# jan-frost/uzliti_slam

Hardware: AMD Instinct MI355X
Metric: SE(3) edges optimized/sec (node-pairs matched/sec in `secondary`) (higher is better)
Workload: dtype f64; 1 GPU; BASELINE config 2: 1000-node / 5000-edge SE(3) pose graph, 20 LM iterations, Huber(1) on loop closures; one independent graph per GPU; system_edges=4999

## Files before the change

### uzliti_slam_amd/csrc/pgo_handle.hpp

```cpp
#pragma once
#include "uzl_common.hpp"
#include "pgo_types.hpp"
#include "pgo_schur.hpp"
#include "pgo_ml_plan.hpp"
#include "pgo_structure.hpp"
#include "pgo_lm.hpp"

#include <algorithm>
#include <chrono>
#include <cstdlib>
#include <cmath>
#include <functional>
#include <limits>
#include <new>
#include <numeric>

namespace uzl {
void k_prepare_nodes(const uzl_node* nodes, int n, int xy, double* pose, hipStream_t s);
void k_prepare_flat_nodes(const double* poses12, int n, double* pose, hipStream_t s);
void k_prepare_edges(const uzl_edge* edges, const int32_t* src, int e, const double* sensors, int ns, int xy, int odom_params,
                     double* zinv, double* info, hipStream_t s);
void k_prepare_flat_edges(const double* meas12, const double* info36, int e, double* zinv, double* info, hipStream_t s);
int k_chi2(const PgoDev& D, const double* pose, double delta, hipStream_t s);
int k_chi2_trial(const PgoDev& D, const double* pose, double delta, hipStream_t s);
// ... 20 lines not shown
void k_edge_error(const PgoDev& D, const double* pose, double* err, hipStream_t s);
void k_poses_out(const double* pose, int n, double* out12, hipStream_t s);
void k_schur_gather(const PgoDev& D, const SchurDev& S, hipStream_t s);
void k_lm_head(const LmSlot* slots, int nslots, int pass_flags, hipStream_t s);
void k_lm_tail(const LmSlot* slots, int nslots, hipStream_t s);
hipError_t kl_linearize(const LmSlot* sl, int nslots, int g_edges, int g_asm, hipStream_t s);
void kl_eval(const LmSlot* sl, int nslots, int g_edges, int g_oplus, hipStream_t s);
void kl_schur_reduce(const LmSlot* sl, const LmShape& sh, hipStream_t s);
void kl_schur_backsub(const LmSlot* sl, const LmShape& sh, hipStream_t s);
void kl_schur_reduce(const HostSlot& hs, const LmShape& sh, hipStream_t s, KernelTimer* timer);
void kl_schur_backsub(const HostSlot& hs, const LmShape& sh, hipStream_t s, KernelTimer* timer);
void kl_ml_numeric(const LmSlot* sl, const LmShape& sh, int which, hipStream_t s);
void kl_ml_trial(const LmSlot* sl, const LmShape& sh, int which, int ns_steps, hipStream_t s);
void kl_ml_numeric(const HostSlot& hs, const LmShape& sh, hipStream_t s, KernelTimer* timer, const std::function<void()>& level1_done);
void kl_ml_trial(const HostSlot& hs, const LmShape& sh, int ns_steps, hipStream_t s, KernelTimer* timer);
void ml_cg_variant(const MlHot& ml, int agg, size_t lds_full, int32_t* variant, int32_t* comp_u, uint64_t* lds);
hipError_t kl_ml_init(const LmSlot* sl, const LmSlot* by_value, const LmShape& sh, int ix, hipStream_t s);
hipError_t kl_ml_pcg_its(const LmSlot* sl, const LmSlot* by_value, const LmShape& sh, int ix, double tol2, int first, int n, hipStream_t s, hipEvent_t* ev = nullptr);
void kl_ml_pcg_init(const HostSlot& hs, const LmShape& sh, hipStream_t s);
void kl_ml_spmv(const HostSlot& hs, const LmShape& sh, int parity, hipStream_t s, hipEvent_t ev_a = nullptr, hipEvent_t ev_b = nullptr);
hipError_t kl_ml_cg(const HostSlot& hs, const LmShape& sh, int parity, int init, hipStream_t s, hipEvent_t ev_a = nullptr, hipEvent_t ev_b = nullptr);
}



namespace uzl { struct LmRun; }
using namespace uzl;

struct SysBufs {
    DevBuf<int32_t> row_ptr, col, rowhdr, b2v;
// ... 75 lines not shown
    struct MlBuf {
        MlDev* dml = nullptr;
        MlHot hot;
        double* rg[2] = {nullptr, nullptr};
        double* y1 = nullptr; double* nsT = nullptr; double* nsX = nullptr;
        double* l1_span_ptr = nullptr;
        hipGraph_t graph = nullptr; hipGraphExec_t graph_exec = nullptr;
        hipGraph_t graph_s = nullptr; hipGraphExec_t graph_exec_s = nullptr;
        double lambda_setup = 0.;
    } mlb[2];
    double* ml_dense_ptr[2][kMlMaxLevels + 1] = {};
    int ml_ix = 0;
    bool ml_pending = false;
    hipStream_t stream2 = nullptr;
    bool streams_borrowed = false;
    hipEvent_t ev_lin = nullptr, ev_setup = nullptr;
    DevBuf<double> d_scal2;
    double lambda_now = 0.;
    DevBuf<uint8_t> ml_arena;
    size_t ml_copy_stride = 0;
    DevBuf<MlDev> d_ml;
    bool no_graph = false;
    int32_t rank = 0, world = 1;
    uzl_allreduce_fn allreduce = nullptr;
    void* allreduce_user = nullptr;
    void* rccl_comm = nullptr;
    bool sharded = false;
    DevBuf<double> d_red;
    int64_t iter_span = 0;
    int64_t l1_span = 0;
    double structure_ms = 0., exchange_ms = 0.;
// ... 17 lines not shown
inline double pgo_eps_t(const uzl_pgo_cfg& c) { return c.pcg_stop == 1 ? 0. : kStepT * c.pcg_tol; }
inline double pgo_eps_r(const uzl_pgo_cfg& c) { return c.pcg_stop == 1 ? 0. : kStepR * c.pcg_tol; }
void build_structure(uzl_pgo* h);
void ensure_structure(uzl_pgo* h);
void destroy_pcg_graph(uzl_pgo* h);
bool ml_async_level(const uzl_pgo* h);
double ml_rate_drop(const uzl_pgo* h);
int ml_ns_steps_at(int structure_steps, int lm_iteration);
void prepare_optimize(uzl_pgo* h);
void own_streams(uzl_pgo* h, bool drain_borrowed);
int do_optimize_host(uzl_pgo* h, int32_t iterations, uzl_pgo_stats* st);
int do_optimize(uzl_pgo* h, int32_t iterations, uzl_pgo_stats* st);
HostSlot host_slot(uzl_pgo* h);
void set_lambda(uzl_pgo* h, double lambda, double tol_f2);
void ml_setup_numeric(uzl_pgo* h, const HostSlot& hs, hipStream_t s, KernelTimer* timer);
int pcg_solve(uzl_pgo* h, int it, bool* converged);
inline double tol_factor2(const uzl_pgo_cfg& c) { return pgo_tol_f2(c); }
struct LmRun;
void lm_run_destroy(LmRun* r);
bool lm_eligible(const uzl_pgo* h);
int do_optimize_lm(uzl_pgo* h, int32_t iterations, uzl_pgo_stats* st);
bool lm_batch_eligible(const std::vector<uzl_pgo*>& hs);
LmSlot make_slot(const uzl_pgo* h, LmDev* d_lm, LmHost* d_pub);
LmShape make_shape(const std::vector<uzl_pgo*>& hs, int nslots, bool batch_geometry);
int batch_optimize_lm(LmRun*& R, const std::vector<uzl_pgo*>& hs, int resident, hipStream_t s, hipStream_t s2, int32_t iterations, bool eager, bool verbose, KernelTimer* timer,
                      uzl_pgo_stats* stats, int* rc_all);
constexpr int kSchurStrongOneMax = 256;
extern const int kUpperNs;
constexpr double kRefreshRel = 1e-3;
constexpr double kRefreshRelSync = 3e-2;
constexpr double kLambdaRetake = 32.;
// ... 4 lines not shown
```

### uzliti_slam_amd/csrc/pgo_ml_kernels.hip

```cpp
#include <hip/hip_ext.h>
#include <functional>
#include <mutex>
#include <type_traits>

#include "pgo_device.hpp"
#include "uzl_common.hpp"

namespace uzl {

#ifdef UZL_STAMPS
__device__ unsigned long long g_stamps[64];
#define STAMP_DECL unsigned long long st_prev_ = __builtin_amdgcn_s_memrealtime(); int st_i_ = 0;
#define STAMP(base) do { if (blockIdx.x == 0 && threadIdx.x == 0) { unsigned long long n_ = __builtin_amdgcn_s_memrealtime(); \
        atomicAdd(&g_stamps[(base) + st_i_], n_ - st_prev_); st_prev_ = n_; } st_i_++; } while (0)
#else
#define STAMP_DECL
#define STAMP(base) do { } while (0)
#endif

struct P3 { double X[9], Y[9], Z[9]; };

__device__ __forceinline__ void mat3(const double* A, const double* B, double* C)
{
#pragma unroll
// ... 2126 lines not shown
    const int B = sh.nslots;
    if (timer) timer->begin("ml_geometry", s);
    if (sh.n_lv[1] <= kGeoAllMax) hipLaunchKernelGGL(ml_geometry_lm_kernel<SLOT>, dim3(1, 1, B), dim3(kBlk), 0, s, sl, which, 0);
    else
        for (int l = 1; l <= sh.levels; l++)
            hipLaunchKernelGGL(ml_geometry_lm_kernel<SLOT>, dim3((sh.n_lv[l] + kBlk - 1) / kBlk, 1, B), dim3(kBlk), 0, s, sl, which, l);
    if (timer) timer->end(s);
    for (int f = 0; f < sh.levels; f++) {
        if (timer) timer->begin("ml_galerkin", s);
        if (sh.chunks[f + 1] > 0) hipLaunchKernelGGL(ml_galerkin_lm_kernel<SLOT>, dim3(sh.chunks[f + 1], 1, B), dim3(kBlk), 0, s, sl, which, f);
        if (timer) timer->end(s);
        if (f == 0 && level1_done) level1_done();
    }
}
template <class SLOT>
static void kl_ml_trial_t(SLOT sl, const LmShape& sh, int which, int ns_steps, hipStream_t s, KernelTimer* timer)
{
    const int B = sh.nslots, L = sh.levels, cl = sh.cl;
    if (timer) timer->begin("ml_sibling", s);
    hipLaunchKernelGGL(ml_inverses_lm_kernel<SLOT>, dim3((sh.inner_aggs + kSibPerBlk - 1) / kSibPerBlk + 1, 1, B), dim3(kBlk), 0, s, sl, which);
    if (timer) timer->end(s);
    if (cl == 0) return;
    const int n6c = 6 * sh.n_lv[cl];
    const long work32 = (long)n6c * (((n6c + 3) & ~3) >> 2);
    if (timer) timer->begin("ml_dense", s);
    if (!sh.mult) {
        for (int l = L - 1; l >= cl; l--)
            hipLaunchKernelGGL(ml_dense_level_lm_kernel<SLOT>, dim3((sh.n_lv[l] * sh.n_lv[l] + kBlk - 1) / kBlk, 1, B), dim3(kBlk), 0, s, sl, which, l);
        hipLaunchKernelGGL(ml_cmat32_lm_kernel<SLOT>, dim3((unsigned)((work32 + kBlk - 1) / kBlk), 1, B), dim3(kBlk), 0, s, sl, which, cl);
        if (timer) timer->end(s);
        return;
    }
    for (int l = L - 1; l >= cl; l--) {
        const int n1 = sh.n_lv[l], n2 = sh.n_lv[l + 1];
        hipLaunchKernelGGL(ml_mult_pair_lm_kernel<SLOT>, dim3(n2 * n2, 1, B), dim3(kBlk), 0, s, sl, which, l);
        const int g12r = (n1 * n2 * 6 + kBlk - 1) / kBlk;
// ... 2 lines not shown
        hipLaunchKernelGGL(ml_mult_qyqt_lm_kernel<SLOT>, dim3(gt * (gt + 1) / 2, 1, B), dim3(256), 0, s, sl, which, l);
        if (l == cl && timer) timer->end(s);
        const int steps = l > cl ? sh.upper_ns : ns_steps;
        for (int k = 0; k < steps; k++) {
            hipLaunchKernelGGL(ml_ns_ax_lm_kernel<SLOT>, dim3(B == 1 ? kXcds * n1 * ax_parts(n6) : n1 * ((n6 + kBlk - 1) / kBlk), 1, B), dim3(kBlk), 0, s, sl, which, l, k);
            const int last = (l == cl && k == steps - 1) ? 1 : 0;
            hipEvent_t ea = nullptr, eb = nullptr;
            if (l == cl && timer) timer->pair("ml_ns_gemm", &ea, &eb);
            if (B == 1 && n6 <= kGemm32Max) launch(ml_ns_gemm32_lm_kernel<SLOT>, dim3(gemm32_grid((n6 + 31) / 32), 1, 1), dim3(256), 0, s, ea, eb, sl, which, l, k, last);
            else launch(ml_ns_gemm_lm_kernel<SLOT>, dim3(gt * (gt + 1) / 2, 1, B), dim3(256), 0, s, ea, eb, sl, which, l, k, last);
        }
    }
    if (ns_steps == 0) hipLaunchKernelGGL(ml_cmat32_lm_kernel<SLOT>, dim3((unsigned)((work32 + kBlk - 1) / kBlk), 1, B), dim3(kBlk), 0, s, sl, which, cl);
}
void kl_ml_numeric(const LmSlot* sl, const LmShape& sh, int which, hipStream_t s) { kl_ml_numeric_t(sl, sh, which, s, nullptr, {}); }
void kl_ml_trial(const LmSlot* sl, const LmShape& sh, int which, int ns_steps, hipStream_t s) { kl_ml_trial_t(sl, sh, which, ns_steps, s, nullptr); }
void kl_ml_numeric(const HostSlot& hs, const LmShape& sh, hipStream_t s, KernelTimer* timer, const std::function<void()>& level1_done)
{
    kl_ml_numeric_t(hs, sh, 0, s, timer, level1_done);
}
void kl_ml_trial(const HostSlot& hs, const LmShape& sh, int ns_steps, hipStream_t s, KernelTimer* timer) { kl_ml_trial_t(hs, sh, 0, ns_steps, s, timer); }

template <class SLOT> __device__ __forceinline__ const LmDev* state_of(const LmSlot& S, const SLOT&) { return S.lm; }
__device__ __forceinline__ const HostSlot* state_of(const LmSlot&, const HostSlot& hs) { return &hs; }
__device__ __forceinline__ bool init_due(const LmDev* lm) { return lm->phase == kLmSolve && lm->init_pass == lm->pass; }
__device__ __forceinline__ bool init_due(const HostSlot*) { return true; }

template <class T>
__device__ __forceinline__ const T* moved(const T* p, int64_t bytes) { return p ? reinterpret_cast<const T*>(reinterpret_cast<const char*>(p) + bytes) : nullptr; }
__device__ __forceinline__ MlHot hot_of(const LmSlot& S, int ix)
{
    MlHot H = S.hot[0];
    const int64_t off = ix ? S.copy_stride : 0;
    H.geo0 = moved(H.geo0, off); H.top_inv = moved(H.top_inv, off); H.Cmat = moved(H.Cmat, off); H.Cmat32 = moved(H.Cmat32, off);
    H.Vg = const_cast<double*>(moved(const_cast<const double*>(H.Vg), off));
#pragma unroll
// ... 327 lines not shown
```

### uzliti_slam_amd/csrc/uzl_pgo.hip

```cpp
#include "pgo_handle.hpp"
#include "pgo_lm.hpp"
#include "uzl_streams.hpp"

#include <array>

using namespace uzl;

#include <dlfcn.h>
#include <exception>
#include <system_error>
#include <thread>
namespace {
struct RcclApi {
    typedef struct { char internal[UZL_RCCL_UNIQUE_ID_BYTES]; } UniqueId;
    typedef void* Comm;
    int (*GetUniqueId)(UniqueId*) = nullptr;
    int (*CommInitRank)(Comm*, int, UniqueId, int) = nullptr;
    int (*CommDestroy)(Comm) = nullptr;
    int (*CommCount)(Comm, int*) = nullptr;
    int (*AllReduce)(const void*, void*, size_t, int, int, Comm, hipStream_t) = nullptr;
    const char* (*GetErrorString)(int) = nullptr;
    static constexpr int kDouble = 8, kSum = 0;
    bool ok = false;
    std::string error;
// ... 298 lines not shown
    const auto t0 = std::chrono::steady_clock::now();
    UZL_HIP(hipStreamBeginCapture(h->stream, hipStreamCaptureModeThreadLocal));
    enqueue_pcg_pairs(h, kGraphPairs, false);
    UZL_HIP(hipStreamEndCapture(h->stream, &B.graph));
    UZL_HIP(hipGraphInstantiate(&B.graph_exec, B.graph, nullptr, nullptr, 0));
    UZL_HIP(hipStreamBeginCapture(h->stream, hipStreamCaptureModeThreadLocal));
    enqueue_pcg_pairs(h, kShortPairs, false);
    UZL_HIP(hipStreamEndCapture(h->stream, &B.graph_s));
    UZL_HIP(hipGraphInstantiate(&B.graph_exec_s, B.graph_s, nullptr, nullptr, 0));
    if (h->cfg.verbose) fprintf(stderr, "[uzl_pgo] structure: %-28s %.3f ms\n", "PCG graphs of one copy", std::chrono::duration<double, std::milli>(std::chrono::steady_clock::now() - t0).count());
    h->structure_ms += std::chrono::duration<double, std::milli>(std::chrono::steady_clock::now() - t0).count();
}

}

int uzl::pcg_solve(uzl_pgo* h, int it, bool* converged)
{
    hipStream_t s = h->stream;
    const PgoDev& D = h->Dp;
    if (D.nb == 0) { *converged = true; h->prev_pcg_iters = 0; h->last_residual_ratio = 0.; return 0; }
    const int max_it = h->cfg.pcg_max_iter > 0 ? h->cfg.pcg_max_iter : 6 * std::max(D.nb, 1);
    const bool timed = h->timer.on || h->no_graph || h->sharded;
    if (h->mlp.levels > 0) {
        const HostSlot hs = host_slot(h);
        if (h->ml_trial_setup) {
            kl_ml_trial(hs, h->ml_shape, ml_ns_steps_at(h->ml_ns_steps, it), s, &h->timer);
            h->ml_trial_setup = false;
            h->mlb[h->ml_ix].lambda_setup = h->lambda_now;
        }
        { Timed t(h, "pcg_init"); kl_ml_pcg_init(hs, h->ml_shape, s); }
        { Timed t(h, "ml_cg"); UZL_HIP(kl_ml_cg(hs, h->ml_shape, 0, 1, s)); }
// ... 5 lines not shown
    int launched = 0;
    constexpr int kFirstPct = 95;
    constexpr int kStep = 2 * kShortPairs;
    const int kLong = 2 * kGraphPairs;
    auto round_up = [](int v) { return ((v + kStep - 1) / kStep) * kStep; };
    int want = h->prev_pcg_iters > 0 ? std::max(kStep, round_up((h->prev_pcg_iters * kFirstPct) / 100 + 1)) : kLong;
    for (int round = 0;; round++) {
        want = round_up(std::max(1, std::min(want, max_it - launched)));
        if (timed) enqueue_pcg_pairs(h, want / 2, h->timer.on);
        else {
            for (int i = 0; i < want / kLong; i++) UZL_HIP(hipGraphLaunch(h->mlb[h->ml_ix].graph_exec, s));
            for (int i = 0; i < (want % kLong + kStep - 1) / kStep; i++) UZL_HIP(hipGraphLaunch(h->mlb[h->ml_ix].graph_exec_s, s));
        }
        launched += want;
        k_residual_guard(D, s);
        fetch_scal(h);
        if (h->h_scal.p->flags[0] || launched >= max_it) break;
        want = round < 2 ? kStep : kLong;
    }
    UZL_HIP(hipGetLastError());
    *converged = h->h_scal.p->flags[0] != 0 && h->h_scal.p->flags[2] == 0;
    h->last_residual_ratio = h->h_scal.p->scal[7];
    if (*converged && (h->ml_mult || h->ml_ns_steps > 0) && !(h->last_residual_ratio <= kResidualGuard)) { *converged = false; h->guard_trips++; }
    const int iters = h->h_scal.p->flags[1];
    h->prev_pcg_iters = iters;
    return iters;
}


namespace uzl {
// ... 231 lines not shown
        uzl_pgo* h;
        ~DrainRebuild() { if (h->ml_pending) { (void)hipStreamSynchronize(h->stream2); h->ml_pending = false; } }
    } drain{h};
    static const bool phases_on = diag_flag("UZL_PHASES");
    std::vector<hipEvent_t> ph_ev;
    std::vector<int> ph_tag;
    auto mark = [&](int tag) {
        if (!phases_on) return;
        hipEvent_t e; if (hipEventCreate(&e) != hipSuccess) return;
        (void)hipEventRecord(e, s); ph_ev.push_back(e); ph_tag.push_back(tag);
    };
    for (int it = 0; it < iterations; it++) {
        int gl, ga;
        adopted = false;
        mark(0);
        if (h->ml_pending) {
            UZL_HIP(hipStreamWaitEvent(s, h->ev_setup, 0));
            h->ml_ix ^= 1; h->ml_pending = false; adopted = true;
        }
        D.pose = h->cur; D.pose_trial = h->trial;
        Dp.pose = h->cur; Dp.pose_trial = h->trial;
        {
            hipEvent_t ea = nullptr, eb = nullptr;
            h->timer.pair("linearize", &ea, &eb);
            UZL_HIP(k_hessian(D, h->cur, delta, &gl, &ga, s, it == 0 || h->sharded, ea, eb));
        }
        if (h->sharded) {
            shard_allreduce(h, h->sys.hdiag.p, (int64_t)h->nb * 42);
            ga = k_diagmax(D, s);
        }
        { Timed t(h, "finalize"); k_finalize(D, gl, 0, ga, 2, s); }
        shard_allreduce_chi2(h);
        const bool refresh = lm_refresh(it, iterations, !async_ok, last_rel, ml_async_level(h) ? kRefreshRel : kRefreshRelSync, rate_ref, rate_last, ml_rate_drop(h));
        bool launch_async = false;
        bool fetched = false;
        if (red) {
            if (h->sharded && SD.runblk) {
                k_schur_gather(D, SD, s);
                shard_allreduce(h, SD.runblk, (int64_t)(SD.n_int + SD.n_runs) * 36);
            }
            if (it == 0) {
// ... 10 lines not shown
            S.precond_builds++;
            if (it == 0 || !async_ok) {
                if (h->mlp.levels > 0) ml_setup_numeric(h, host_slot(h), s, &h->timer);
                h->ml_trial_setup = true;
            } else launch_async = true;
        }
        if ((it == 0 || h->sharded) && !fetched) {
            fetch_scal(h);
            current_chi = h->h_scal.p->scal[4];
        }
        if (it == 0 && !fetched) {
            S.chi2_initial = current_chi;
            lambda = 1e-5 * h->h_scal.p->scal[6];
            ni = 2.;
        }
        if (launch_async) {
            const int nb_ix = h->ml_ix ^ 1;
            UZL_HIP(hipEventRecord(h->ev_lin, s));
            UZL_HIP(hipStreamWaitEvent(h->stream2, h->ev_lin, 0));
            HostSlot hb = host_slot(h);
            hb.ix = nb_ix;
            hb.S.Dp.scal = h->d_scal2.p;
            k_set_scalar(hb.S.Dp.scal + 3, lambda, h->stream2);
            ml_setup_numeric(h, hb, h->stream2, nullptr);
            kl_ml_trial(hb, h->ml_shape, h->ml_ns_steps, h->stream2, nullptr);
            h->mlb[nb_ix].lambda_setup = lambda;
            UZL_HIP(hipEventRecord(h->ev_setup, h->stream2));
            h->ml_pending = true;
        }
        double rho = 0.;
        int qmax = 0;
        const double tol_f2 = tol_factor2(h->cfg);
        mark(1);
        do {
            set_lambda(h, lambda, tol_f2);
            if (red && qmax > 0) {
                if (h->ml_pending) UZL_HIP(hipStreamWaitEvent(s, h->ev_setup, 0));
                schur_reduce();
            }
            bool conv = false;
            if (h->mlp.levels > 0 && lambda > kLambdaRetake * h->mlb[h->ml_ix].lambda_setup) h->ml_trial_setup = true;
            const bool fresh = h->ml_trial_setup || (adopted && qmax == 0);
            int pcg_its = pcg_solve(h, it, &conv);
            S.pcg_iterations += pcg_its;
            if (!conv && !fresh && h->mlp.levels > 0) {
                h->ml_trial_setup = true;
                pcg_its = pcg_solve(h, it, &conv);
                S.pcg_iterations += pcg_its;
            }
            if (!conv && (h->ml_mult || h->ml_ns_steps > 0)) {
                if (h->cfg.verbose)
                    fprintf(stderr, "[uzl_pgo] it %d trial %d lambda %.3e: multiplicative operator refused (pcg %d, rz %.3e, breakdown %d, |r|2/|b|2 %.3e) -> additive\n",
                            it, qmax, lambda, pcg_its, h->h_scal.p->scal[0], (int)h->h_scal.p->flags[2], h->last_residual_ratio);
                if (h->ml_pending) {
                    UZL_HIP(hipStreamSynchronize(h->stream2));
                    h->ml_pending = false; last_rel = 1e300;
                }
                h->ml_mult = false; h->ml_ns_steps = 0; h->mult_banned = true;
// ... 100 lines not shown
    if (cfg) c = *cfg; else uzl_pgo_cfg_default(&c);
    if (check_device(c.device) != UZL_OK) return UZL_ERR_NO_DEVICE;
    uzl_pgo* h = new (std::nothrow) uzl_pgo();
    if (!h) return UZL_ERR_OOM;
    h->cfg = c;
    memset(&h->D, 0, sizeof(h->D));
    { const char* ng = getenv("UZL_NO_GRAPH"); h->no_graph = ng && ng[0] == '1'; }
    if (getenv("UZL_VERBOSE")) h->cfg.verbose = 1;
    bool ok = hipSetDevice(c.device) == hipSuccess;
    if (ok && shared) { h->stream = shared; h->stream2 = shared2; h->streams_borrowed = true; }
    else if (ok) {
        h->stream = stream_lease(c.device, 0, {}, false);
        h->stream2 = h->stream ? stream_lease(c.device, -1, {h->stream}, false) : nullptr;
        ok = h->stream && h->stream2;
    }
    ok = ok && hipEventCreateWithFlags(&h->ev_lin, hipEventDisableTiming) == hipSuccess && hipEventCreateWithFlags(&h->ev_setup, hipEventDisableTiming) == hipSuccess;
    if (!ok) {
        if (!h->streams_borrowed) { stream_release(c.device, h->stream); stream_release(c.device, h->stream2); }
        if (h->ev_lin) (void)hipEventDestroy(h->ev_lin);
        if (h->ev_setup) (void)hipEventDestroy(h->ev_setup);
        delete h;
        return UZL_ERR_HIP;
    }
    *out = h;
    return UZL_OK;
}
void uzl::own_streams(uzl_pgo* h, bool drain_borrowed)
{
    if (!h->streams_borrowed) return;
    UZL_HIP(hipSetDevice(h->cfg.device));
    if (drain_borrowed) {
        UZL_HIP(hipStreamSynchronize(h->stream));
        if (h->stream2) UZL_HIP(hipStreamSynchronize(h->stream2));
    }
// ... 27 lines not shown
    cfg->pass_history = 0;
}

int uzl_pgo_create(const uzl_pgo_cfg* cfg, uzl_pgo** out) { return pgo_create_on(cfg, nullptr, nullptr, out); }

void uzl_pgo_destroy(uzl_pgo* h)
{
    if (!h) return;
    (void)hipSetDevice(h->cfg.device);
    if (h->stream) (void)hipStreamSynchronize(h->stream);
    if (h->stream2) (void)hipStreamSynchronize(h->stream2);
    destroy_pcg_graph(h);
    lm_run_destroy(h->lm); h->lm = nullptr;
    if (h->rccl_comm) { (void)rccl().CommDestroy(h->rccl_comm); h->rccl_comm = nullptr; }
    if (h->ev_lin) (void)hipEventDestroy(h->ev_lin);
    if (h->ev_setup) (void)hipEventDestroy(h->ev_setup);
    if (!h->streams_borrowed) { stream_release(h->cfg.device, h->stream2); stream_release(h->cfg.device, h->stream); }
    delete h;
}

int uzl_pgo_set_config(uzl_pgo* h, const uzl_pgo_cfg* cfg)
{
    if (!h || !cfg) return UZL_ERR_BAD_ARG;
    std::lock_guard<std::mutex> lock(h->mu);
    if (cfg->device != h->cfg.device) return fail(h, UZL_ERR_BAD_ARG, "device cannot change after create");
    if (cfg->iterations < 1 || cfg->pcg_tol <= 0. || cfg->huber_delta <= 0.) return fail(h, UZL_ERR_BAD_ARG, "bad config value");
    if (cfg->pcg_tol != h->cfg.pcg_tol) destroy_pcg_graph(h);
    if (cfg->preconditioner != h->cfg.preconditioner || cfg->schur_reduce != h->cfg.schur_reduce || cfg->reduced_numbering != h->cfg.reduced_numbering) h->structure_ready = false;
    h->cfg = *cfg;
    return UZL_OK;
// ... 440 lines not shown
```

### uzliti_slam_amd/csrc/uzl_pgo_lm.hip

```cpp
#include "pgo_handle.hpp"

namespace uzl {

struct LmRun {
    int nslots = 0;
    DevBuf<LmSlot> d_slots;
    DevBuf<LmDev> d_lm;
    PinBuf<LmHost> h_pub;
    LmHost* d_pub = nullptr;
    PinBuf<LmDev> h_init;
    std::vector<LmSlot> slots;
    LmShape shape{};
    DevBuf<double> d_start;
    hipEvent_t ev_fork = nullptr, ev_join = nullptr;
    bool join_pending = false;
    uint64_t gen = ~0ull;
    int solves_of_gen = 0;
    int first_solve_its = 0;
    std::vector<std::vector<int>> trial_its_prev, trial_its_cur;
    std::vector<uint64_t> hist_gen;
    struct Seg { hipGraph_t g = nullptr; hipGraphExec_t x = nullptr; };
    Seg setup, reb, pcg_long[2];
    void drop(Seg& q) { if (q.x) { (void)hipGraphExecDestroy(q.x); q.x = nullptr; } if (q.g) { (void)hipGraphDestroy(q.g); q.g = nullptr; } }
    void drop_all() { drop(setup); drop(reb); drop(pcg_long[0]); drop(pcg_long[1]); }
};

void lm_run_destroy(LmRun* r)
{
    if (!r) return;
    r->drop_all();
    if (r->ev_fork) (void)hipEventDestroy(r->ev_fork);
    if (r->ev_join) (void)hipEventDestroy(r->ev_join);
    delete r;
}

namespace {

LmRun* new_run()
{
    LmRun* R = new LmRun();
    if (hipEventCreateWithFlags(&R->ev_fork, hipEventDisableTiming) != hipSuccess || hipEventCreateWithFlags(&R->ev_join, hipEventDisableTiming) != hipSuccess) {
        lm_run_destroy(R);
        throw HipError{hipErrorUnknown, "hipEventCreate", __FILE__, __LINE__};
    }
    return R;
}
void reserve_slots(LmRun* R, int n)
{
    R->nslots = n;
    R->d_slots.reserve((size_t)n); R->d_lm.reserve((size_t)n);
    R->h_pub.reserve((size_t)n, hipHostMallocMapped | hipHostMallocCoherent);
    R->h_init.reserve((size_t)n);
    UZL_HIP(hipHostGetDevicePointer((void**)&R->d_pub, R->h_pub.p, 0));
    R->slots.resize((size_t)n);
}

void enq_linearize(LmRun* R, hipStream_t s)
{
    const LmShape& sh = R->shape;
    UZL_HIP(kl_linearize(R->d_slots.p, sh.nslots, sh.g_edges, sh.g_asm, s));
}
void enq_head(LmRun* R, int pass_flags, bool linearized, hipStream_t s)
{
    const LmShape& sh = R->shape;
    if (!linearized) enq_linearize(R, s);
    k_lm_head(R->d_slots.p, sh.nslots, pass_flags, s);
    if (sh.red) kl_schur_reduce(R->d_slots.p, sh, s);
}
void enq_setup(LmRun* R, int which, int ns_steps, hipStream_t s)
// ... 89 lines not shown

LmDev initial_state(const uzl_pgo* h, int iterations)
{
    LmDev I;
    memset(&I, 0, sizeof(I));
    I.flags[0] = 1;
    I.phase = kLmLin; I.cur = 0; I.ix = 0;
    I.init_pass = I.schur_pass = I.numeric_pass = I.trial_pass = I.build_pass = -1;
    I.iterations = iterations;
    I.max_it = h->cfg.pcg_max_iter > 0 ? h->cfg.pcg_max_iter : 6 * std::max(h->Dp.nb, 1);
    I.sync_rebuild = ml_async_level(h) ? 0 : 1;
    I.guarded = (h->ml_mult || h->ml_ns_steps > 0) ? 1 : 0;
    I.ni = 2.; I.last_rel = 1e300; I.rate_ref = -1.; I.rate_last = -1.;
    I.tol_f2 = pgo_tol_f2(h->cfg); I.eps_t = pgo_eps_t(h->cfg); I.eps_r = pgo_eps_r(h->cfg);
    I.refresh_rel = ml_async_level(h) ? kRefreshRel : kRefreshRelSync; I.rate_drop = ml_rate_drop(h); I.tol2 = h->cfg.pcg_tol * h->cfg.pcg_tol; I.lambda_retake = kLambdaRetake; I.delta = h->cfg.huber_delta;
    return I;
}
LmDev idle_state()
{
    LmDev I;
    memset(&I, 0, sizeof(I));
    I.flags[0] = 1; I.phase = kLmDone;
    I.init_pass = I.schur_pass = I.numeric_pass = I.trial_pass = I.build_pass = -1;
    return I;
}

uint32_t wait_pub(hipStream_t s, LmRun* R, int sl, uint32_t seq, LmHost* out)
{
    const auto t0 = std::chrono::steady_clock::now();
    volatile LmHost* pub = R->h_pub.p + sl;
// ... 50 lines not shown
            UZL_HIP(hipMemcpyAsync(h->pose_a.p, h->cur, sizeof(double) * 8 * (size_t)h->n, hipMemcpyDeviceToDevice, s));
            h->cur = h->pose_a.p; h->trial = h->pose_b.p;
        }
        UZL_HIP(hipMemcpyAsync(R->d_start.p + j.start_off, h->cur, sizeof(double) * 8 * (size_t)h->n, hipMemcpyDeviceToDevice, s));
    }
    std::vector<int> slot_job((size_t)nS, -1), solve_passes((size_t)nS, 0), prev_last((size_t)nS, 0), seen_trials((size_t)nS, 0), cur_last((size_t)nS, 0);
    std::vector<uint32_t> sent((size_t)nS, 0);
    std::vector<LmHost> snap((size_t)nS);
    int next_job = 0, n_active = 0;
    auto load_slot = [&](int sl, bool first) {
        LmDev I;
        if (next_job < Q) {
            const int j = next_job++;
            slot_job[sl] = j;
            R->slots[sl] = make_slot(jobs[j].h, R->d_lm.p + sl, R->d_pub + sl);
            UZL_HIP(hipMemcpyAsync(R->d_slots.p + sl, &R->slots[sl], sizeof(LmSlot), hipMemcpyHostToDevice, s));
            I = initial_state(jobs[j].h, o.iterations);
            n_active++;
        } else {
            slot_job[sl] = -1;
            I = idle_state();
        }
        if (first) { memset(R->h_pub.p + sl, 0, sizeof(LmHost)); sent[sl] = 0; }
        I.tails = (int32_t)sent[sl];
        R->h_init.p[sl] = I;
        UZL_HIP(hipMemcpyAsync(R->d_lm.p + sl, R->h_init.p + sl, sizeof(LmDev), hipMemcpyHostToDevice, s));
        memset(&snap[sl], 0, sizeof(LmHost));
        snap[sl].lm = I;
        solve_passes[sl] = 0; prev_last[sl] = 0; cur_last[sl] = 0; seen_trials[sl] = 0;
    };
    for (int sl = 0; sl < nS; sl++) load_slot(sl, true);
// ... 2 lines not shown
        bool same = R->hist_gen.size() == (size_t)Q;
        for (int j = 0; same && j < Q; j++) same = R->hist_gen[(size_t)j] == jobs[(size_t)j].h->structure_gen;
        if (same) R->trial_its_prev.swap(R->trial_its_cur); else R->trial_its_prev.clear();
        R->trial_its_prev.resize((size_t)Q);
        R->trial_its_cur.assign((size_t)Q, std::vector<int>());
        R->hist_gen.resize((size_t)Q);
        for (int j = 0; j < Q; j++) R->hist_gen[(size_t)j] = jobs[(size_t)j].h->structure_gen;
    }
    struct Drain {
        LmRun* R; hipStream_t s2;
        ~Drain() { if (R->join_pending) { (void)hipStreamSynchronize(s2); R->join_pending = false; } }
    } drain{R, o.s2};
    static const bool phases_on = diag_flag("UZL_PHASES");
    std::vector<hipEvent_t> ph_ev;
    std::vector<int> ph_tag;
    auto mark = [&](int tag) {
        if (!phases_on) return;
        hipEvent_t e; if (hipEventCreate(&e) != hipSuccess) return;
        (void)hipEventRecord(e, s); ph_ev.push_back(e); ph_tag.push_back(tag);
    };
    int passes = 0;
    double enq_ms = 0., wait_ms = 0.;
    bool lin_ahead = false;
    while (n_active > 0) {
        const auto tp0 = std::chrono::steady_clock::now();
        int pf = 0, want = 0;
        bool any_start = false;
        for (int sl = 0; sl < nS; sl++) {
            if (slot_job[sl] < 0 || jobs[slot_job[sl]].finished) continue;
            const LmDev& v = snap[sl].lm;
// ... 27 lines not shown
        const int base = (nS == 1 && slot_job[0] >= 0 && snap[0].lm.phase == kLmSolve) ? snap[0].lm.flags[1] : 0;
        static const bool wrong_ix = diag_flag("UZL_LM_WRONG_IX");
        const int pass_ix = lm_pass_ix(snap[0].lm.phase, snap[0].lm.ix, snap[0].lm.pending) ^ (wrong_ix ? 1 : 0);
        const double tol2 = snap[0].lm.tol2;
        mark(0);
        if (any_start && R->join_pending) { UZL_HIP(hipStreamWaitEvent(s, R->ev_join, 0)); R->join_pending = false; }
        mark(1);
        if (any_start) enq_head(R, pf, lin_ahead, s);
        lin_ahead = false;
        mark(2);
        if (pf & kPassSetup) {
            const int steps = nS == 1 ? ml_ns_steps_at(R->shape.ns_steps, snap[0].lm.it) : R->shape.ns_steps;
            if (steps != R->shape.ns_steps) enq_setup(R, 1, steps, s);
            else run_seg(R->setup, eager, s, [&](hipStream_t q) { enq_setup(R, 1, steps, q); });
        }
        if (pf & kPassRebuild) {
            UZL_HIP(hipEventRecord(R->ev_fork, s));
            UZL_HIP(hipStreamWaitEvent(o.s2, R->ev_fork, 0));
            run_seg(R->reb, eager, o.s2, [&](hipStream_t q) { enq_setup(R, 0, R->shape.ns_steps, q); });
            UZL_HIP(hipEventRecord(R->ev_join, o.s2));
            R->join_pending = true;
        }
        mark(3);
        if (any_start) enq_init(R, pass_ix, s);
        mark(4);
        if (o.timer && o.timer->on) {
            std::vector<hipEvent_t> ev((size_t)4 * want);
            for (int q = 0; q < want; q++) { o.timer->pair(o.spmv_name, &ev[4 * q], &ev[4 * q + 1]); o.timer->pair(o.cg_name, &ev[4 * q + 2], &ev[4 * q + 3]); }
            enq_pcg(R, pass_ix, tol2, base, want, s, ev.data());
        } else {
            int first = base, left = want;
            if (!eager && (first & 1)) { enq_pcg(R, pass_ix, tol2, first, 1, s); first++; left--; }
            const int n_long = eager ? 0 : left / kLong, rem = left - n_long * kLong;
            for (int i = 0; i < n_long; i++) run_seg(R->pcg_long[pass_ix], false, s, [&](hipStream_t q) { enq_pcg(R, pass_ix, tol2, 0, kLong, q); });
            if (rem > 0) enq_pcg(R, pass_ix, tol2, first + n_long * kLong, rem, s);
        }
        mark(5);
        enq_tail(R, s);
        if (!R->join_pending && !(o.timer && o.timer->on)) { enq_linearize(R, s); lin_ahead = true; }
        mark(6);
        passes++;
        for (int sl = 0; sl < nS; sl++) sent[sl]++;
        const auto tp1 = std::chrono::steady_clock::now();
        if (o.verbose) fprintf(stderr, "[uzl_pgo]   pass %d enqueued: segments %d, %d PCG iterations, %d graph(s) in the slots\n", passes - 1, pf, want, n_active);
        bool refill = false;
        for (int sl = 0; sl < nS; sl++) {
            if (slot_job[sl] < 0 || jobs[slot_job[sl]].finished) continue;
            (void)wait_pub(s, R, sl, sent[sl], &snap[sl]);
            LmJob& J = jobs[slot_job[sl]];
            const LmDev& v = snap[sl].lm;
            J.passes++;
            if (o.verbose)
                fprintf(stderr, "[uzl_pgo] pass %d, graph %d -> it %d trial %d phase %d: pcg %d done %d (last solve %d) lambda %.3e chi2 %.9g |r|2/|b|2 %.3e need %d\n", passes - 1,
                        slot_job[sl], v.it, v.qmax, v.phase, v.flags[1], v.flags[0], v.pcg_last, v.lambda, v.chi_cur, snap[sl].scal[7], v.need);
            if (v.st_lm_trials > seen_trials[sl]) { seen_trials[sl] = v.st_lm_trials; prev_last[sl] = cur_last[sl]; cur_last[sl] = v.pcg_last; }
            if (v.st_lm_trials == 1 && v.pcg_last > 0 && slot_job[sl] == 0) R->first_solve_its = v.pcg_last;
            {
                std::vector<int>& cur = R->trial_its_cur[(size_t)slot_job[sl]];
                if (v.st_lm_trials > 0 && (size_t)v.st_lm_trials > cur.size()) cur.resize((size_t)v.st_lm_trials, v.pcg_last);
            }
            if (v.phase == kLmDone || v.phase == kLmAnomaly) {
                J.last = snap[sl]; J.finished = true; J.anomaly = v.phase == kLmAnomaly;
                n_active--; refill = true;
            }
        }
        if (o.timer && o.timer->on) { UZL_HIP(hipStreamSynchronize(s)); o.timer->resolve(); }
// ... 2 lines not shown
            for (int sl = 0; sl < nS; sl++)
                if (slot_job[sl] >= 0 && jobs[slot_job[sl]].finished) load_slot(sl, false);
            lin_ahead = false;
        }
        const auto tp2 = std::chrono::steady_clock::now();
        enq_ms += std::chrono::duration<double, std::milli>(tp1 - tp0).count(); wait_ms += std::chrono::duration<double, std::milli>(tp2 - tp1).count();
    }
    UZL_HIP(hipGetLastError());
    if (o.verbose) fprintf(stderr, "[uzl_pgo] device-resident loop: %d passes, host time enqueueing %.3f ms, waiting for snapshots %.3f ms\n", passes, enq_ms, wait_ms);
    if (R->join_pending) { UZL_HIP(hipStreamSynchronize(o.s2)); R->join_pending = false; }
    UZL_HIP(hipStreamSynchronize(s));
    if (phases_on && ph_ev.size() > 1) {
        double acc[7] = {0, 0, 0, 0, 0, 0, 0};
        static const char* nm[7] = {"wait for the rebuild (0->1)", "linearise + head (1->2)", "set-up / fork (2->3)", "init (3->4)", "pcg (4->5)", "tail (5->6)", "between passes (6->0)"};
        static const bool each = diag_flag("UZL_PHASES_EACH");
        for (size_t i = 0; i + 1 < ph_ev.size(); i++) {
            float ms = 0.f; (void)hipEventElapsedTime(&ms, ph_ev[i], ph_ev[i + 1]); acc[ph_tag[i] % 7] += ms;
            if (each) fprintf(stderr, "%s%d:%.0f", ph_tag[i] == 0 ? "\n[uzl_pgo]   " : " ", ph_tag[i], 1e3 * ms);
        }
        if (each) fprintf(stderr, "\n");
        fprintf(stderr, "[uzl_pgo] segments over %d passes (GPU event time, ms):", passes);
        for (int k = 0; k < 7; k++) fprintf(stderr, "  %s %.3f", nm[k], acc[k]);
        fprintf(stderr, "\n");
        for (hipEvent_t e : ph_ev) (void)hipEventDestroy(e);
    }
    return passes;
}

void finish_job(LmJob& J, uzl_pgo_stats* st, double wall_ms)
{
    uzl_pgo* h = J.h;
    const LmDev& v = J.last.lm;
    h->cur = v.cur ? h->pose_b.p : h->pose_a.p; h->trial = v.cur ? h->pose_a.p : h->pose_b.p;
// ... 113 lines not shown
```

### uzliti_slam_amd/csrc/uzl_streams.hip

```cpp
#include "uzl_streams.hpp"

#include <algorithm>
#include <chrono>

namespace uzl {
namespace {

constexpr int kPoolMax = 16;
constexpr int kNewPerLease = 6;
constexpr int kMaxDevices = 16;
constexpr int kKeepFree = 32;

__global__ void chain_kernel(unsigned ticks, unsigned long long* stamp, int where, int slot)
{
    const unsigned long long t0 = wall_clock64();
    if (where == 1 && blockIdx.x == 0 && threadIdx.x == 0) stamp[2 * slot] = t0;
    while (wall_clock64() - t0 < ticks) {}
    if (where == 2 && (blockIdx.x & 63) == 63 && threadIdx.x == 0) atomicMax(&stamp[2 * slot + 1], wall_clock64());
}

__global__ void stamps_out_kernel(const unsigned long long* __restrict__ stamp, unsigned long long* __restrict__ host, unsigned long long seq, int n)
{
    if ((int)threadIdx.x < n) __hip_atomic_store(&host[threadIdx.x], stamp[threadIdx.x], __ATOMIC_RELAXED, __HIP_MEMORY_SCOPE_SYSTEM);
    __threadfence_system();
// ... 13 lines not shown
    unsigned long long* host = nullptr;
    unsigned long long seq = 0;
    hipEvent_t ev[kGroupMax] = {nullptr, nullptr, nullptr, nullptr};
    double alone = 0.;
    double warm_ms = 0.;
    std::vector<hipStream_t> warmed;
};

double chain_ticks(Probe& pr, const hipStream_t* q, int n)
{
    if (!pr.stamp) {
        const auto t_init = std::chrono::steady_clock::now();
        struct Done { Probe& p; std::chrono::steady_clock::time_point t; ~Done() { p.warm_ms += std::chrono::duration<double, std::milli>(std::chrono::steady_clock::now() - t).count(); } } done{pr, t_init};
        if (hipMalloc((void**)&pr.stamp, 2 * kGroupMax * sizeof(unsigned long long)) != hipSuccess) { pr.stamp = nullptr; return -1.; }
        if (hipMemset(pr.stamp, 0, 2 * kGroupMax * sizeof(unsigned long long)) != hipSuccess) return -1.;
        if (hipHostMalloc((void**)&pr.host, (2 * kGroupMax + 1) * sizeof(unsigned long long), hipHostMallocDefault) != hipSuccess) { pr.host = nullptr; return -1.; }
        pr.host[2 * kGroupMax] = 0;
        for (hipEvent_t& e : pr.ev) if (hipEventCreateWithFlags(&e, hipEventDisableTiming) != hipSuccess) { e = nullptr; return -1.; }
        hipLaunchKernelGGL(chain_kernel, dim3(1), dim3(64), 0, q[0], 1u, pr.stamp, 0, 0);
        hipLaunchKernelGGL(stamps_out_kernel, dim3(1), dim3(64), 0, q[0], pr.stamp, pr.host, 0ull, 2 * kGroupMax);
        (void)hipStreamSynchronize(q[0]);
        pr.warmed.push_back(q[0]);
    }
    if (!pr.host || n < 1 || n > kGroupMax) return -1.;
    for (int i = 0; i < n; i++)
        if (std::find(pr.warmed.begin(), pr.warmed.end(), q[i]) == pr.warmed.end()) {
            const auto t0 = std::chrono::steady_clock::now();
            hipLaunchKernelGGL(chain_kernel, dim3(1), dim3(64), 0, q[i], 1u, pr.stamp, 0, 0);
            (void)hipStreamSynchronize(q[i]);
            pr.warmed.push_back(q[i]);
            pr.warm_ms += std::chrono::duration<double, std::milli>(std::chrono::steady_clock::now() - t0).count();
// ... 268 lines not shown
```

Baseline: 18.92 million edges/s.

## Split ML rebuild into inverses and dense phases to overlap with linearize and PCG

```diff
diff --git a/uzliti_slam_amd/csrc/pgo_handle.hpp b/uzliti_slam_amd/csrc/pgo_handle.hpp
--- a/uzliti_slam_amd/csrc/pgo_handle.hpp
+++ b/uzliti_slam_amd/csrc/pgo_handle.hpp
@@ -58,6 +58,10 @@
 void kl_ml_trial(const LmSlot* sl, const LmShape& sh, int which, int ns_steps, hipStream_t s);
 void kl_ml_numeric(const HostSlot& hs, const LmShape& sh, hipStream_t s, KernelTimer* timer, const std::function<void()>& level1_done);
 void kl_ml_trial(const HostSlot& hs, const LmShape& sh, int ns_steps, hipStream_t s, KernelTimer* timer);
+void kl_ml_inverses(const LmSlot* sl, const LmShape& sh, int which, hipStream_t s);
+void kl_ml_dense(const LmSlot* sl, const LmShape& sh, int which, int ns_steps, hipStream_t s);
+void kl_ml_inverses(const HostSlot& hs, const LmShape& sh, hipStream_t s);
+void kl_ml_dense(const HostSlot& hs, const LmShape& sh, int ns_steps, hipStream_t s);
 void ml_cg_variant(const MlHot& ml, int agg, size_t lds_full, int32_t* variant, int32_t* comp_u, uint64_t* lds);
 hipError_t kl_ml_init(const LmSlot* sl, const LmSlot* by_value, const LmShape& sh, int ix, hipStream_t s);
 hipError_t kl_ml_pcg_its(const LmSlot* sl, const LmSlot* by_value, const LmShape& sh, int ix, double tol2, int first, int n, hipStream_t s, hipEvent_t* ev = nullptr);
@@ -163,7 +167,7 @@
     bool ml_pending = false;
     hipStream_t stream2 = nullptr;
     bool streams_borrowed = false;
-    hipEvent_t ev_lin = nullptr, ev_setup = nullptr;
+    hipEvent_t ev_lin = nullptr, ev_hfree = nullptr, ev_setup = nullptr;
     DevBuf<double> d_scal2;
     double lambda_now = 0.;
     DevBuf<uint8_t> ml_arena;
@@ -211,7 +215,7 @@
 HostSlot host_slot(uzl_pgo* h);
 void set_lambda(uzl_pgo* h, double lambda, double tol_f2);
 void ml_setup_numeric(uzl_pgo* h, const HostSlot& hs, hipStream_t s, KernelTimer* timer);
-int pcg_solve(uzl_pgo* h, int it, bool* converged);
+int pcg_solve(uzl_pgo* h, int it, bool* converged, const std::function<void()>& behind_first_batch = {});
 inline double tol_factor2(const uzl_pgo_cfg& c) { return pgo_tol_f2(c); }
 struct LmRun;
 void lm_run_destroy(LmRun* r);
diff --git a/uzliti_slam_amd/csrc/pgo_ml_kernels.hip b/uzliti_slam_amd/csrc/pgo_ml_kernels.hip
--- a/uzliti_slam_amd/csrc/pgo_ml_kernels.hip
+++ b/uzliti_slam_amd/csrc/pgo_ml_kernels.hip
@@ -2164,12 +2164,16 @@
     }
 }
 template <class SLOT>
-static void kl_ml_trial_t(SLOT sl, const LmShape& sh, int which, int ns_steps, hipStream_t s, KernelTimer* timer)
+static void kl_ml_inverses_t(SLOT sl, const LmShape& sh, int which, hipStream_t s, KernelTimer* timer)
+{
+    if (timer) timer->begin("ml_sibling", s);
+    hipLaunchKernelGGL(ml_inverses_lm_kernel<SLOT>, dim3((sh.inner_aggs + kSibPerBlk - 1) / kSibPerBlk + 1, 1, sh.nslots), dim3(kBlk), 0, s, sl, which);
+    if (timer) timer->end(s);
+}
+template <class SLOT>
+static void kl_ml_dense_t(SLOT sl, const LmShape& sh, int which, int ns_steps, hipStream_t s, KernelTimer* timer)
 {
     const int B = sh.nslots, L = sh.levels, cl = sh.cl;
-    if (timer) timer->begin("ml_sibling", s);
-    hipLaunchKernelGGL(ml_inverses_lm_kernel<SLOT>, dim3((sh.inner_aggs + kSibPerBlk - 1) / kSibPerBlk + 1, 1, B), dim3(kBlk), 0, s, sl, which);
-    if (timer) timer->end(s);
     if (cl == 0) return;
     const int n6c = 6 * sh.n_lv[cl];
     const long work32 = (long)n6c * (((n6c + 3) & ~3) >> 2);
@@ -2202,12 +2206,16 @@
     if (ns_steps == 0) hipLaunchKernelGGL(ml_cmat32_lm_kernel<SLOT>, dim3((unsigned)((work32 + kBlk - 1) / kBlk), 1, B), dim3(kBlk), 0, s, sl, which, cl);
 }
 void kl_ml_numeric(const LmSlot* sl, const LmShape& sh, int which, hipStream_t s) { kl_ml_numeric_t(sl, sh, which, s, nullptr, {}); }
-void kl_ml_trial(const LmSlot* sl, const LmShape& sh, int which, int ns_steps, hipStream_t s) { kl_ml_trial_t(sl, sh, which, ns_steps, s, nullptr); }
+void kl_ml_trial(const LmSlot* sl, const LmShape& sh, int which, int ns_steps, hipStream_t s) { kl_ml_inverses_t(sl, sh, which, s, nullptr); kl_ml_dense_t(sl, sh, which, ns_steps, s, nullptr); }
+void kl_ml_inverses(const LmSlot* sl, const LmShape& sh, int which, hipStream_t s) { kl_ml_inverses_t(sl, sh, which, s, nullptr); }
+void kl_ml_dense(const LmSlot* sl, const LmShape& sh, int which, int ns_steps, hipStream_t s) { kl_ml_dense_t(sl, sh, which, ns_steps, s, nullptr); }
+void kl_ml_inverses(const HostSlot& hs, const LmShape& sh, hipStream_t s) { kl_ml_inverses_t(hs, sh, 0, s, nullptr); }
+void kl_ml_dense(const HostSlot& hs, const LmShape& sh, int ns_steps, hipStream_t s) { kl_ml_dense_t(hs, sh, 0, ns_steps, s, nullptr); }
 void kl_ml_numeric(const HostSlot& hs, const LmShape& sh, hipStream_t s, KernelTimer* timer, const std::function<void()>& level1_done)
 {
     kl_ml_numeric_t(hs, sh, 0, s, timer, level1_done);
 }
-void kl_ml_trial(const HostSlot& hs, const LmShape& sh, int ns_steps, hipStream_t s, KernelTimer* timer) { kl_ml_trial_t(hs, sh, 0, ns_steps, s, timer); }
+void kl_ml_trial(const HostSlot& hs, const LmShape& sh, int ns_steps, hipStream_t s, KernelTimer* timer) { kl_ml_inverses_t(hs, sh, 0, s, timer); kl_ml_dense_t(hs, sh, 0, ns_steps, s, timer); }
 
 template <class SLOT> __device__ __forceinline__ const LmDev* state_of(const LmSlot& S, const SLOT&) { return S.lm; }
 __device__ __forceinline__ const HostSlot* state_of(const LmSlot&, const HostSlot& hs) { return &hs; }
diff --git a/uzliti_slam_amd/csrc/uzl_pgo.hip b/uzliti_slam_amd/csrc/uzl_pgo.hip
--- a/uzliti_slam_amd/csrc/uzl_pgo.hip
+++ b/uzliti_slam_amd/csrc/uzl_pgo.hip
@@ -336,7 +336,7 @@
 
 }
 
-int uzl::pcg_solve(uzl_pgo* h, int it, bool* converged)
+int uzl::pcg_solve(uzl_pgo* h, int it, bool* converged, const std::function<void()>& behind_first_batch)
 {
     hipStream_t s = h->stream;
     const PgoDev& D = h->Dp;
@@ -372,6 +372,7 @@
         }
         launched += want;
         k_residual_guard(D, s);
+        if (round == 0 && behind_first_batch) behind_first_batch();
         fetch_scal(h);
         if (h->h_scal.p->flags[0] || launched >= max_it) break;
         want = round < 2 ? kStep : kLong;
@@ -633,9 +634,10 @@
         int gl, ga;
         adopted = false;
         mark(0);
-        if (h->ml_pending) {
-            UZL_HIP(hipStreamWaitEvent(s, h->ev_setup, 0));
-            h->ml_ix ^= 1; h->ml_pending = false; adopted = true;
+        const bool join_due = h->ml_pending;
+        if (join_due) {
+            UZL_HIP(hipStreamWaitEvent(s, h->ev_hfree, 0));
+            h->ml_ix ^= 1; adopted = true;
         }
         D.pose = h->cur; D.pose_trial = h->trial;
         Dp.pose = h->cur; Dp.pose_trial = h->trial;
@@ -644,6 +646,7 @@
             h->timer.pair("linearize", &ea, &eb);
             UZL_HIP(k_hessian(D, h->cur, delta, &gl, &ga, s, it == 0 || h->sharded, ea, eb));
         }
+        if (join_due) { UZL_HIP(hipStreamWaitEvent(s, h->ev_setup, 0)); h->ml_pending = false; }
         if (h->sharded) {
             shard_allreduce(h, h->sys.hdiag.p, (int64_t)h->nb * 42);
             ga = k_diagmax(D, s);
@@ -684,19 +687,25 @@
             lambda = 1e-5 * h->h_scal.p->scal[6];
             ni = 2.;
         }
+        std::function<void()> fork_rebuild;
         if (launch_async) {
-            const int nb_ix = h->ml_ix ^ 1;
             UZL_HIP(hipEventRecord(h->ev_lin, s));
-            UZL_HIP(hipStreamWaitEvent(h->stream2, h->ev_lin, 0));
-            HostSlot hb = host_slot(h);
-            hb.ix = nb_ix;
-            hb.S.Dp.scal = h->d_scal2.p;
-            k_set_scalar(hb.S.Dp.scal + 3, lambda, h->stream2);
-            ml_setup_numeric(h, hb, h->stream2, nullptr);
-            kl_ml_trial(hb, h->ml_shape, h->ml_ns_steps, h->stream2, nullptr);
-            h->mlb[nb_ix].lambda_setup = lambda;
-            UZL_HIP(hipEventRecord(h->ev_setup, h->stream2));
-            h->ml_pending = true;
+            fork_rebuild = [h, lambda]() {
+                const int nb_ix = h->ml_ix ^ 1;
+                UZL_HIP(hipStreamWaitEvent(h->stream2, h->ev_lin, 0));
+                HostSlot hb = host_slot(h);
+                hb.ix = nb_ix;
+                hb.S.Dp.scal = h->d_scal2.p;
+                k_set_scalar(hb.S.Dp.scal + 3, lambda, h->stream2);
+                ml_setup_numeric(h, hb, h->stream2, nullptr);
+                kl_ml_inverses(hb, h->ml_shape, h->stream2);
+                UZL_HIP(hipEventRecord(h->ev_hfree, h->stream2));
+                kl_ml_dense(hb, h->ml_shape, h->ml_ns_steps, h->stream2);
+                h->mlb[nb_ix].lambda_setup = lambda;
+                UZL_HIP(hipEventRecord(h->ev_setup, h->stream2));
+                h->ml_pending = true;
+            };
+            if (h->no_graph) { fork_rebuild(); fork_rebuild = nullptr; }
         }
         double rho = 0.;
         int qmax = 0;
@@ -711,7 +720,9 @@
             bool conv = false;
             if (h->mlp.levels > 0 && lambda > kLambdaRetake * h->mlb[h->ml_ix].lambda_setup) h->ml_trial_setup = true;
             const bool fresh = h->ml_trial_setup || (adopted && qmax == 0);
-            int pcg_its = pcg_solve(h, it, &conv);
+            int pcg_its = pcg_solve(h, it, &conv, fork_rebuild);
+            if (fork_rebuild && !h->ml_pending) fork_rebuild();
+            fork_rebuild = nullptr;
             S.pcg_iterations += pcg_its;
             if (!conv && !fresh && h->mlp.levels > 0) {
                 h->ml_trial_setup = true;
@@ -842,10 +853,12 @@
         h->stream2 = h->stream ? stream_lease(c.device, -1, {h->stream}, false) : nullptr;
         ok = h->stream && h->stream2;
     }
-    ok = ok && hipEventCreateWithFlags(&h->ev_lin, hipEventDisableTiming) == hipSuccess && hipEventCreateWithFlags(&h->ev_setup, hipEventDisableTiming) == hipSuccess;
+    ok = ok && hipEventCreateWithFlags(&h->ev_lin, hipEventDisableTiming) == hipSuccess && hipEventCreateWithFlags(&h->ev_hfree, hipEventDisableTiming) == hipSuccess &&
+         hipEventCreateWithFlags(&h->ev_setup, hipEventDisableTiming) == hipSuccess;
     if (!ok) {
         if (!h->streams_borrowed) { stream_release(c.device, h->stream); stream_release(c.device, h->stream2); }
         if (h->ev_lin) (void)hipEventDestroy(h->ev_lin);
+        if (h->ev_hfree) (void)hipEventDestroy(h->ev_hfree);
         if (h->ev_setup) (void)hipEventDestroy(h->ev_setup);
         delete h;
         return UZL_ERR_HIP;
@@ -903,6 +916,7 @@
     lm_run_destroy(h->lm); h->lm = nullptr;
     if (h->rccl_comm) { (void)rccl().CommDestroy(h->rccl_comm); h->rccl_comm = nullptr; }
     if (h->ev_lin) (void)hipEventDestroy(h->ev_lin);
+    if (h->ev_hfree) (void)hipEventDestroy(h->ev_hfree);
     if (h->ev_setup) (void)hipEventDestroy(h->ev_setup);
     if (!h->streams_borrowed) { stream_release(h->cfg.device, h->stream2); stream_release(h->cfg.device, h->stream); }
     delete h;
diff --git a/uzliti_slam_amd/csrc/uzl_pgo_lm.hip b/uzliti_slam_amd/csrc/uzl_pgo_lm.hip
--- a/uzliti_slam_amd/csrc/uzl_pgo_lm.hip
+++ b/uzliti_slam_amd/csrc/uzl_pgo_lm.hip
@@ -12,8 +12,10 @@
     std::vector<LmSlot> slots;
     LmShape shape{};
     DevBuf<double> d_start;
-    hipEvent_t ev_fork = nullptr, ev_join = nullptr;
+    hipEvent_t ev_fork = nullptr, ev_hfree = nullptr, ev_join = nullptr;
     bool join_pending = false;
+    std::vector<LmSlot> slots_sent;
+    std::vector<uint8_t> slot_valid;
     uint64_t gen = ~0ull;
     int solves_of_gen = 0;
     int first_solve_its = 0;
@@ -30,6 +32,7 @@
     if (!r) return;
     r->drop_all();
     if (r->ev_fork) (void)hipEventDestroy(r->ev_fork);
+    if (r->ev_hfree) (void)hipEventDestroy(r->ev_hfree);
     if (r->ev_join) (void)hipEventDestroy(r->ev_join);
     delete r;
 }
@@ -39,7 +42,8 @@
 LmRun* new_run()
 {
     LmRun* R = new LmRun();
-    if (hipEventCreateWithFlags(&R->ev_fork, hipEventDisableTiming) != hipSuccess || hipEventCreateWithFlags(&R->ev_join, hipEventDisableTiming) != hipSuccess) {
+    if (hipEventCreateWithFlags(&R->ev_fork, hipEventDisableTiming) != hipSuccess || hipEventCreateWithFlags(&R->ev_hfree, hipEventDisableTiming) != hipSuccess ||
+        hipEventCreateWithFlags(&R->ev_join, hipEventDisableTiming) != hipSuccess) {
         lm_run_destroy(R);
         throw HipError{hipErrorUnknown, "hipEventCreate", __FILE__, __LINE__};
     }
@@ -53,6 +57,7 @@
     R->h_init.reserve((size_t)n);
     UZL_HIP(hipHostGetDevicePointer((void**)&R->d_pub, R->h_pub.p, 0));
     R->slots.resize((size_t)n);
+    R->slots_sent.resize((size_t)n); R->slot_valid.assign((size_t)n, 0);
 }
 
 void enq_linearize(LmRun* R, hipStream_t s)
@@ -172,6 +177,8 @@
     I.ni = 2.; I.last_rel = 1e300; I.rate_ref = -1.; I.rate_last = -1.;
     I.tol_f2 = pgo_tol_f2(h->cfg); I.eps_t = pgo_eps_t(h->cfg); I.eps_r = pgo_eps_r(h->cfg);
     I.refresh_rel = ml_async_level(h) ? kRefreshRel : kRefreshRelSync; I.rate_drop = ml_rate_drop(h); I.tol2 = h->cfg.pcg_tol * h->cfg.pcg_tol; I.lambda_retake = kLambdaRetake; I.delta = h->cfg.huber_delta;
+    static const bool skip_rebuilds = diag_flag("UZL_LM_SKIP_REBUILD");
+    if (skip_rebuilds && !I.sync_rebuild) { I.refresh_rel = 1e300; I.rate_drop = 0.; }
     return I;
 }
 LmDev idle_state()
@@ -252,7 +259,13 @@
             const int j = next_job++;
             slot_job[sl] = j;
             R->slots[sl] = make_slot(jobs[j].h, R->d_lm.p + sl, R->d_pub + sl);
-            UZL_HIP(hipMemcpyAsync(R->d_slots.p + sl, &R->slots[sl], sizeof(LmSlot), hipMemcpyHostToDevice, s));
+            static const bool always_send = diag_flag("UZL_LM_SLOT_RESEND");
+            if (always_send || !R->slot_valid[sl] || memcmp(&R->slots_sent[sl], &R->slots[sl], sizeof(LmSlot)) != 0) {
+                R->slot_valid[sl] = 0;
+                UZL_HIP(hipMemcpyAsync(R->d_slots.p + sl, &R->slots[sl], sizeof(LmSlot), hipMemcpyHostToDevice, s));
+                memcpy(&R->slots_sent[sl], &R->slots[sl], sizeof(LmSlot));
+                R->slot_valid[sl] = 1;
+            }
             I = initial_state(jobs[j].h, o.iterations);
             n_active++;
         } else {
@@ -285,6 +298,7 @@
     static const bool phases_on = diag_flag("UZL_PHASES");
     std::vector<hipEvent_t> ph_ev;
     std::vector<int> ph_tag;
+    std::vector<int> ph_reb, ph_its;
     auto mark = [&](int tag) {
         if (!phases_on) return;
         hipEvent_t e; if (hipEventCreate(&e) != hipSuccess) return;
@@ -342,12 +356,21 @@
             if (steps != R->shape.ns_steps) enq_setup(R, 1, steps, s);
             else run_seg(R->setup, eager, s, [&](hipStream_t q) { enq_setup(R, 1, steps, q); });
         }
-        if (pf & kPassRebuild) {
-            UZL_HIP(hipEventRecord(R->ev_fork, s));
+        static const bool fork_first_sw = diag_flag("UZL_LM_FORK_FIRST");
+        const bool fork_first = fork_first_sw || eager;
+        auto enq_rebuild = [&]() {
             UZL_HIP(hipStreamWaitEvent(o.s2, R->ev_fork, 0));
-            run_seg(R->reb, eager, o.s2, [&](hipStream_t q) { enq_setup(R, 0, R->shape.ns_steps, q); });
+            kl_ml_numeric(R->d_slots.p, R->shape, 0, o.s2);
+            kl_ml_inverses(R->d_slots.p, R->shape, 0, o.s2);
+            UZL_HIP(hipEventRecord(R->ev_hfree, o.s2));
+            if (R->shape.cl > 0) run_seg(R->reb, eager, o.s2, [&](hipStream_t q) { kl_ml_dense(R->d_slots.p, R->shape, 0, R->shape.ns_steps, q); });
             UZL_HIP(hipEventRecord(R->ev_join, o.s2));
             R->join_pending = true;
+        };
+        const bool rebuild = (pf & kPassRebuild) != 0;
+        if (rebuild) {
+            UZL_HIP(hipEventRecord(R->ev_fork, s));
+            if (fork_first) enq_rebuild();
         }
         mark(3);
         if (any_start) enq_init(R, pass_ix, s);
@@ -364,9 +387,15 @@
             if (rem > 0) enq_pcg(R, pass_ix, tol2, first + n_long * kLong, rem, s);
         }
         mark(5);
+        if (rebuild && !fork_first) enq_rebuild();
         enq_tail(R, s);
-        if (!R->join_pending && !(o.timer && o.timer->on)) { enq_linearize(R, s); lin_ahead = true; }
+        static const bool lin_waits_join = diag_flag("UZL_LM_LIN_WAITS_JOIN");
+        if (!(o.timer && o.timer->on) && !(R->join_pending && lin_waits_join)) {
+            if (R->join_pending) UZL_HIP(hipStreamWaitEvent(s, R->ev_hfree, 0));
+            enq_linearize(R, s); lin_ahead = true;
+        }
         mark(6);
+        if (phases_on) ph_reb.push_back(rebuild ? want : -want);
         passes++;
         for (int sl = 0; sl < nS; sl++) sent[sl]++;
         const auto tp1 = std::chrono::steady_clock::now();
@@ -378,6 +407,7 @@
             LmJob& J = jobs[slot_job[sl]];
             const LmDev& v = snap[sl].lm;
             J.passes++;
+            if (phases_on && sl == 0) ph_its.push_back(v.phase == kLmSolve ? v.flags[1] : v.pcg_last);
             if (o.verbose)
                 fprintf(stderr, "[uzl_pgo] pass %d, graph %d -> it %d trial %d phase %d: pcg %d done %d (last solve %d) lambda %.3e chi2 %.9g |r|2/|b|2 %.3e need %d\n", passes - 1,
                         slot_job[sl], v.it, v.qmax, v.phase, v.flags[1], v.flags[0], v.pcg_last, v.lambda, v.chi_cur, snap[sl].scal[7], v.need);
@@ -410,9 +440,14 @@
         double acc[7] = {0, 0, 0, 0, 0, 0, 0};
         static const char* nm[7] = {"wait for the rebuild (0->1)", "linearise + head (1->2)", "set-up / fork (2->3)", "init (3->4)", "pcg (4->5)", "tail (5->6)", "between passes (6->0)"};
         static const bool each = diag_flag("UZL_PHASES_EACH");
+        size_t pass_no = 0;
         for (size_t i = 0; i + 1 < ph_ev.size(); i++) {
             float ms = 0.f; (void)hipEventElapsedTime(&ms, ph_ev[i], ph_ev[i + 1]); acc[ph_tag[i] % 7] += ms;
-            if (each) fprintf(stderr, "%s%d:%.0f", ph_tag[i] == 0 ? "\n[uzl_pgo]   " : " ", ph_tag[i], 1e3 * ms);
+            if (each && ph_tag[i] == 0 && pass_no < ph_reb.size()) {
+                fprintf(stderr, "\n[uzl_pgo]   %c launches=%d its=%d", ph_reb[pass_no] > 0 ? 'R' : '-', std::abs(ph_reb[pass_no]), pass_no < ph_its.size() ? ph_its[pass_no] : -1);
+                pass_no++;
+            }
+            if (each) fprintf(stderr, " %d:%.0f", ph_tag[i], 1e3 * ms);
         }
         if (each) fprintf(stderr, "\n");
         fprintf(stderr, "[uzl_pgo] segments over %d passes (GPU event time, ms):", passes);
diff --git a/uzliti_slam_amd/csrc/uzl_streams.hip b/uzliti_slam_amd/csrc/uzl_streams.hip
--- a/uzliti_slam_amd/csrc/uzl_streams.hip
+++ b/uzliti_slam_amd/csrc/uzl_streams.hip
@@ -51,7 +51,7 @@
         struct Done { Probe& p; std::chrono::steady_clock::time_point t; ~Done() { p.warm_ms += std::chrono::duration<double, std::milli>(std::chrono::steady_clock::now() - t).count(); } } done{pr, t_init};
         if (hipMalloc((void**)&pr.stamp, 2 * kGroupMax * sizeof(unsigned long long)) != hipSuccess) { pr.stamp = nullptr; return -1.; }
         if (hipMemset(pr.stamp, 0, 2 * kGroupMax * sizeof(unsigned long long)) != hipSuccess) return -1.;
-        if (hipHostMalloc((void**)&pr.host, (2 * kGroupMax + 1) * sizeof(unsigned long long), hipHostMallocDefault) != hipSuccess) { pr.host = nullptr; return -1.; }
+        if (hipHostMalloc((void**)&pr.host, (2 * kGroupMax + 1) * sizeof(unsigned long long), hipHostMallocMapped | hipHostMallocCoherent) != hipSuccess) { pr.host = nullptr; return -1.; }
         pr.host[2 * kGroupMax] = 0;
         for (hipEvent_t& e : pr.ev) if (hipEventCreateWithFlags(&e, hipEventDisableTiming) != hipSuccess) { e = nullptr; return -1.; }
         hipLaunchKernelGGL(chain_kernel, dim3(1), dim3(64), 0, q[0], 1u, pr.stamp, 0, 0);
```

Result: no change. 19.04 million edges/s, median of 6 (+0.7%).
